# autonomousvision/unimatch

Hardware: AMD Instinct MI355X
Metric: image_pairs_per_sec (higher is better)
Workload: dtype f16x2

## Files before the change

### unimatch_amd/build.py

```python
import os
import re
import shutil
import subprocess
import sys

HERE = os.path.dirname(os.path.abspath(__file__))
CSRC = os.path.join(HERE, 'csrc')
LIB = os.path.join(HERE, 'libunimatch_hip.so')
SOURCES = ['capi.hip', 'global_match.hip', 'window_attn.hip', 'local_ops.hip', 'linear.hip', 'ffn.hip', 'conv.hip', 'nhwc_ops.hip', 'norm_ops.hip', 'upsample.hip',
           'rccl_gather.hip', 'local_corr_mfma.hip', 'aliases.hip', 'probe.hip', 'video.hip', 'metrics.hip', 'prepost.hip', 'visualize.hip']
DIAG_SOURCES = ['microbench.hip']
HEADERS = ['common.h', 'planes.h', 'timing.h', os.path.join('..', '..', 'include', 'unimatch_hip.h')]
EXTRA_FLAGS = {'ffn.hip': ['-fno-slp-vectorize'], 'global_match.hip': ['-fno-slp-vectorize', '-mllvm', '-amdgpu-mfma-vgpr-form', '-Wno-inline-asm'], 'window_attn.hip': ['-fno-slp-vectorize'],
               'linear.hip': ['-fno-slp-vectorize'],
               'video.hip': ['-ffp-contract=off'],
               'metrics.hip': ['-ffp-contract=off', '-fhip-fp32-correctly-rounded-divide-sqrt'],
               'prepost.hip': ['-ffp-contract=off', '-fhip-fp32-correctly-rounded-divide-sqrt'],
               'visualize.hip': ['-ffp-contract=off', '-fhip-fp32-correctly-rounded-divide-sqrt']}
RESOURCE_GUARDS = {'conv.hip': {'conv_entry_kernel': 2}}
FLAGS = ['--offload-arch=gfx950', '-O3', '-std=c++17', '-fPIC', '-fno-gpu-rdc', '-Wno-unused-result']


def find_hipcc():
    for cand in (os.environ.get('HIPCC'), shutil.which('hipcc'), '/opt/rocm/bin/hipcc'):
        if cand and os.path.exists(cand):
            return cand
    raise RuntimeError('hipcc not found: the HIP extension cannot be built')


def parse_resource_report(text):
    out, cur = {}, None
    for line in text.splitlines():
        m = re.search(r'remark: .*?Function Name: (\S+)', line)
        if m:
            cur = out.setdefault(m.group(1), {})
            continue
        m = re.search(r'remark: .*?\s{2,}([A-Za-z ]+?)(?: \[[^\]]*\])?: (\d+)', line)
        if m and cur is not None:
            cur[m.group(1).strip()] = int(m.group(2))
    return out


def check_resources(src, report):
    for key, min_occ in RESOURCE_GUARDS.get(src, {}).items():
        hits = {k: v for k, v in report.items() if key in k}
        if not hits:
            raise RuntimeError(f'{src}: no resource report for {key}: the guard of unimatch_amd/build.py has nothing to check')
        for name, r in hits.items():
            if r.get('ScratchSize', -1) != 0 or r.get('Occupancy', 0) < min_occ:
                raise RuntimeError(f'{src}: {name} needs scratch {r.get("ScratchSize")} B/lane at occupancy {r.get("Occupancy")} '
                                   f'({r.get("VGPRs")} VGPRs): it was written for no scratch at {min_occ} waves per SIMD')


def _stale(target, deps):
    if not os.path.exists(target):
        return True
    t = os.path.getmtime(target)
    return any(os.path.getmtime(d) > t for d in deps)


def build(force=False, verbose=False):
    hipcc = find_hipcc()
    objdir = os.path.join(HERE, '_obj')
    os.makedirs(objdir, exist_ok=True)
    hdrs = [os.path.normpath(os.path.join(CSRC, h)) for h in HEADERS] + [os.path.abspath(__file__)]
    objs = []
    for src in SOURCES:
        s = os.path.join(CSRC, src)
        o = os.path.join(objdir, src.replace('.hip', '.o'))
        if force or _stale(o, [s] + hdrs) or (src in RESOURCE_GUARDS and not os.path.exists(o[:-2] + '.resources.txt')):
            cmd = [hipcc] + FLAGS + EXTRA_FLAGS.get(src, []) + ['-c', s, '-o', o]
            if verbose:
                print(' '.join(cmd))
            if src in RESOURCE_GUARDS:
                done = subprocess.run(cmd + ['-Rpass-analysis=kernel-resource-usage', '-fno-caret-diagnostics'], cwd=CSRC, stderr=subprocess.PIPE, text=True)
                remarks = [ln for ln in done.stderr.splitlines() if 'kernel-resource-usage' in ln]
                sys.stderr.write('\n'.join(ln for ln in done.stderr.splitlines() if 'kernel-resource-usage' not in ln))
                if done.returncode != 0:
                    raise subprocess.CalledProcessError(done.returncode, cmd)
                try:
                    check_resources(src, parse_resource_report('\n'.join(remarks)))
                except RuntimeError:
                    os.remove(o)
                    raise
                with open(o[:-2] + '.resources.txt', 'w') as f:
                    f.write('\n'.join(remarks) + '\n')
            else:
                subprocess.run(cmd, check=True, cwd=CSRC)
        objs.append(o)
    if force or _stale(LIB, objs):
        cmd = [hipcc, '--offload-arch=gfx950', '-shared', '-fPIC', '-o', LIB] + objs + ['-ldl']
        if verbose:
            print(' '.join(cmd))
        subprocess.run(cmd, check=True)
    return LIB


def build_variant(name, defines, verbose=False, only=None):
    hipcc = find_hipcc()
    objdir = os.path.join(HERE, '_variants', '_obj_' + name)
    os.makedirs(objdir, exist_ok=True)
    objs = []
    defines = list(defines) + ['-DUM_DIAGNOSTIC_BUILD']
    if only:
        build(verbose=verbose)
    for src in SOURCES + DIAG_SOURCES:
        if only and src not in only and src not in DIAG_SOURCES:
            objs.append(os.path.join(HERE, '_obj', src.replace('.hip', '.o')))
            continue
        o = os.path.join(objdir, src.replace('.hip', '.o'))
        cmd = [hipcc] + FLAGS + EXTRA_FLAGS.get(src, []) + list(defines) + ['-c', os.path.join(CSRC, src), '-o', o]
        if verbose:
            print(' '.join(cmd))
        subprocess.run(cmd, check=True, cwd=CSRC)
        objs.append(o)
    lib = os.path.join(HERE, '_variants', f'lib{name}.so')
    subprocess.run([hipcc, '--offload-arch=gfx950', '-shared', '-fPIC', '-o', lib] + objs + ['-ldl'], check=True)
    shutil.rmtree(objdir, ignore_errors=True)
    return lib


if __name__ == '__main__':
    if '--variant' in sys.argv:
        i = sys.argv.index('--variant')
        only = sys.argv[sys.argv.index('--only') + 1].split(',') if '--only' in sys.argv else None
        print(build_variant(sys.argv[i + 1], [a for a in sys.argv[i + 2:] if a.startswith('-D')], verbose=True, only=only))
    else:
        print(build(force='--force' in sys.argv, verbose=True))
```

### unimatch_amd/csrc/conv.hip

```cpp
#include <cstdlib>
#include <cstring>
#ifndef UM_CONV_2P
#define UM_CONV_2P 0
#endif
#include "common.h"
#include "planes.h"

struct ConvArgs {
    const unsigned short* ap;
    long a_plane_stride;
    unsigned row_stride;
    unsigned zero_row;
    const unsigned short* wp;
    long w_plane_stride;
    const float* bias;
    float* out;
    unsigned short* outp;
    long outp_plane_stride;
    int out_ld, out_coff, outp_ld, outp_coff;
    int act;
    int gate, gate_c, gate_zld;
    float* gate_h;
    const float* gate_z;
    float* gate_hout;
// ... 447 lines not shown
    __syncthreads();

    int ptap = 0, pcc = 0;
    for (int s = 0; s < nstage; ++s) {
        unsigned char* cur = lds + (s & 1) * STAGE;
        unsigned char* nxt = lds + ((s & 1) ^ 1) * STAGE;
        const bool centre = ENTRY && ptap == 4;
        if constexpr (ENTRY) {
            if (centre) proj_load(pcc, 0);
        }
        if (s + 1 < nstage) {
            stage_async(cc * 32, (s + 1) * 32, nxt);
            if constexpr (ENTRY) entry_load(cc * 32);
            advance();
        }
        const unsigned char* at = cur + 32 * wave * 64;
        const unsigned char* wt = cur + NS * TILE;
        __builtin_amdgcn_s_setprio(1);
#pragma unroll
        for (int ks = 0; ks < 2; ++ks) {
            const i16x8 bh = *reinterpret_cast<const i16x8*>(at + foff[ks]);
            i16x8 bl;
            if (NS == 2) bl = *reinterpret_cast<const i16x8*>(at + TILE + foff[ks]);
#pragma unroll
            for (int nt = 0; nt < NT; ++nt) {
                const i16x8 wh = *reinterpret_cast<const i16x8*>(wt + nt * 32 * 64 + foff[ks]);
                if (NS == 2) {
                    const i16x8 wl = *reinterpret_cast<const i16x8*>(wt + WTILE + nt * 32 * 64 + foff[ks]);
                    if (UM_CONV_2P != 1) acc[nt] = T::mfma(wl, bh, acc[nt]);
                    if (UM_CONV_2P != 2) acc[nt] = T::mfma(wh, bl, acc[nt]);
                }
                acc[nt] = T::mfma(wh, bh, acc[nt]);
            }
            if constexpr (ENTRY) {
                if (centre) {
#pragma unroll
                    for (int nt = 0; nt < NT; ++nt) {
                        if (NS == 2) {
                            if (UM_CONV_2P != 1) acc2[nt] = T::mfma(pwl[nt], bh, acc2[nt]);
                            if (UM_CONV_2P != 2) acc2[nt] = T::mfma(pwh[nt], bl, acc2[nt]);
                        }
                        acc2[nt] = T::mfma(pwh[nt], bh, acc2[nt]);
                    }
                    if (ks == 0) proj_load(pcc, 1);
                }
            }
        }
        __builtin_amdgcn_s_setprio(0);
        if constexpr (ENTRY) {
            if (s + 1 < nstage) entry_store(nxt);
            if (++pcc == cpt) {
                pcc = 0;
                ++ptap;
            }
        }
        asm volatile("s_waitcnt vmcnt(0)" ::: "memory");
        __syncthreads();
    }

    {
        const int rloc0 = pl0 + 32 * wave;
        conv_epilogue<T, NS, NT, NT, !ENTRY>(a, acc, lds, lds + RING, bt, rloc0, min(32, max(0, P - rloc0)), bt * ((P + 127) / 128) + pl0 / 128, false,
                                 n0, tid, wave, lane, half);
        if constexpr (ENTRY) {
            ConvArgs a2 = a;
            a2.bias = e.bias2;
            a2.out = e.out2;
            a2.stats = e.stats2;
            __syncthreads();
            conv_epilogue<T, NS, NT, NT, false>(a2, acc2, lds, lds + RING, bt, rloc0, min(32, max(0, P - rloc0)), bt * ((P + 127) / 128) + pl0 / 128,
                                     false, n0, tid, wave, lane, half);
        }
    }
}

template <typename T, int NS, int NT>
__global__ __launch_bounds__(256, 2) void conv_kernel(ConvArgs a) {
    __shared__ __attribute__((aligned(16))) unsigned char lds[ConvLds<NS, NT>::TOTAL];
    conv_body<T, NS, NT, false>(a, ConvEntryArgs{}, lds);
}

template <typename T, int NS, int NT>
__global__ __launch_bounds__(256, 2) void conv_entry_kernel(ConvArgs a, ConvEntryArgs e) {
    __shared__ __attribute__((aligned(16))) unsigned char lds[ConvLds<NS, NT>::ENTRY_TOTAL];
    conv_body<T, NS, NT, true>(a, e, lds);
}

template <int NS, int NT, int KW, int NSLOT>
struct ConvRowsLds {
    static constexpr int NTE = NT < 2 ? NT : 2;
    static constexpr int ATILE = 288 * 32;
    static constexpr int WTILE = 32 * NT * 32;
    static constexpr int STAGE = NS * (ATILE + KW * WTILE);
    static constexpr int EPI = 8 * 32 * (32 * NTE * 4);
    static constexpr int RING = (NSLOT * STAGE > EPI) ? NSLOT * STAGE : EPI;
    static constexpr int TOTAL = RING + 8 * 2 * 32 * NT * 4 + 64;
};

__device__ __forceinline__ void conv_wait_vm(int n) {
    switch (n) {
        case 0: asm volatile("s_waitcnt vmcnt(0)" ::: "memory"); break;
        case 1: asm volatile("s_waitcnt vmcnt(1)" ::: "memory"); break;
        case 2: asm volatile("s_waitcnt vmcnt(2)" ::: "memory"); break;
        case 3: asm volatile("s_waitcnt vmcnt(3)" ::: "memory"); break;
        case 4: asm volatile("s_waitcnt vmcnt(4)" ::: "memory"); break;
        case 6: asm volatile("s_waitcnt vmcnt(6)" ::: "memory"); break;
        case 8: asm volatile("s_waitcnt vmcnt(8)" ::: "memory"); break;
        case 9: asm volatile("s_waitcnt vmcnt(9)" ::: "memory"); break;
        case 12: asm volatile("s_waitcnt vmcnt(12)" ::: "memory"); break;
        case 16: asm volatile("s_waitcnt vmcnt(16)" ::: "memory"); break;
        case 18: asm volatile("s_waitcnt vmcnt(18)" ::: "memory"); break;
        case 24: asm volatile("s_waitcnt vmcnt(24)" ::: "memory"); break;
        default: asm volatile("s_waitcnt vmcnt(0)" ::: "memory"); break;
    }
}

template <typename T, int NS, int NT, int KW, int NSLOT>
__global__ __launch_bounds__(512, (NSLOT == 2 && NT < 4 ? 2 : 1)) void conv_rows_kernel(ConvArgs a) {
    using L = ConvRowsLds<NS, NT, KW, NSLOT>;
    constexpr int ATILE = L::ATILE, WTILE = L::WTILE, STAGE = L::STAGE, RING = L::RING;
    extern __shared__ __attribute__((aligned(16))) unsigned char lds[];

    const int tid = threadIdx.x, lane = tid & 63;
    const int wave = __builtin_amdgcn_readfirstlane(tid >> 6);
    const int half = lane >> 5, fr = lane & 31;
    const int P = a.Ho * a.Wo, tpi = (P + 255) / 256;
    const int ny = (a.Cout + 32 * NT - 1) / (32 * NT);
    const int wg = a.xcd ? xcd_remap(blockIdx.x, gridDim.x) : blockIdx.x;
    const int tile = wg / ny;
    const int bt = tile / tpi, pl0 = (tile - bt * tpi) * 256;
    const int n0 = (wg - tile * ny) * (32 * NT);
    const int cpt = a.Cin >> 4;
    const int nstage = a.KH * cpt;
    const int ktot = a.KH * KW * a.Cin;

    const int dcp = lane & 1;
    int wy[2];
    long wflat[2];
    bool wok[2];
#pragma unroll
    for (int i = 0; i < 2; ++i) {
        const int jr = i == 0 ? wave : 8;
        const int j = 32 * jr + (lane >> 1);
        const int p = pl0 + j - a.pad_w;
        wok[i] = (i == 0 || wave == 7) && p >= 0 && p < P;
        const int rem = wok[i] ? p : 0;
        wy[i] = rem / a.Wo - a.pad_h;
        wflat[i] = (long)bt * P + rem - (long)a.pad_h * a.Wi;
    }
    unsigned rowoff[2];
    auto set_ky = [&](int ky) {
#pragma unroll
        for (int i = 0; i < 2; ++i) {
            const int iy = wy[i] + ky;
            const bool ok = wok[i] && (unsigned)iy < (unsigned)a.Hi;
            const unsigned row = ok ? (unsigned)(wflat[i] + (long)ky * a.Wi) : a.zero_row;
            rowoff[i] = row * a.row_stride;
        }
    };
    constexpr int NPIECE = 2 + (KW * NT + 7) / 8;
    auto stage_piece = [&](int k, int ky, int cc, unsigned char* buf) {
        if (k < 2) {
            const int jr = k == 0 ? wave : 8;
            if (k == 0 || wave == 7) {
                const int r = 32 * jr + (lane >> 1);
                const int sc = dcp ^ ((r >> 3) & 1);
                const unsigned off = rowoff[k] + (unsigned)((cc * 16 + 8 * sc) * 2);
#pragma unroll
                for (int pl = 0; pl < NS; ++pl) conv_dma16(a.ap + pl * a.a_plane_stride, off, buf + pl * ATILE + (32 * jr) * 32);
            }
        } else {
            const int q = wave + 8 * (k - 2);
            if (q < KW * NT) {
                const int kx = q / NT, jb = q - kx * NT;
                const int r = 32 * jb + (lane >> 1);
                const int sc = dcp ^ ((r >> 3) & 1);
                const int n = min(n0 + r, a.Cout - 1);
                const unsigned off = (unsigned)(((long)n * ktot + (ky * KW + kx) * a.Cin + cc * 16 + 8 * sc) * 2);
#pragma unroll
                for (int pl = 0; pl < NS; ++pl)
                    conv_dma16(a.wp + pl * a.w_plane_stride, off, buf + NS * ATILE + (kx * NS + pl) * WTILE + (32 * jb) * 32);
            }
        }
    };

    bool tap_ok[KW];
    bool any_masked = false;
    {
        const int p = pl0 + 32 * wave + fr;
        const bool pok = p < P;
        const int x = (pok ? p : 0) % a.Wo;
#pragma unroll
        for (int kx = 0; kx < KW; ++kx) {
            tap_ok[kx] = pok && (unsigned)(x + kx - a.pad_w) < (unsigned)a.Wi;
            any_masked |= !tap_ok[kx];
        }
    }
    const bool wave_masked = __any(any_masked);

    f32x16 acc[NT];
#pragma unroll
    for (int nt = 0; nt < NT; ++nt)
#pragma unroll
        for (int r = 0; r < 16; ++r) acc[nt][r] = 0.f;

    const int foffw = fr * 32 + ((half ^ ((fr >> 3) & 1)) << 4);
    int foffa[KW];
#pragma unroll
    for (int kx = 0; kx < KW; ++kx) {
        const int r = 32 * wave + fr + kx;
        foffa[kx] = r * 32 + ((half ^ ((r >> 3) & 1)) << 4);
    }

    int cnt = NS * (1 + (wave == 7 ? 1 : 0));
#pragma unroll
    for (int k = 2; k < NPIECE; ++k) cnt += (wave + 8 * (k - 2) < KW * NT) ? NS : 0;
    constexpr int D = NSLOT - 1;

    int ky = 0, cc = 0;
    set_ky(0);
    auto advance = [&]() {
        if (++cc == cpt) {
            cc = 0;
            ++ky;
            set_ky(ky);
        }
    };
#pragma unroll
    for (int d = 0; d < D; ++d)
        if (d < nstage) {
#pragma unroll
            for (int k = 0; k < NPIECE; ++k) stage_piece(k, ky, cc, lds + d * STAGE);
            advance();
        }
    conv_wait_vm(nstage >= D ? cnt * (D - 1) : 0);
    __syncthreads();

    int cur_off = 0, nxt_off = D * STAGE;
    for (int s = 0; s < nstage; ++s) {
        unsigned char* cur = lds + cur_off;
        unsigned char* nxt = lds + nxt_off;
        const bool more = s + D < nstage;
        __builtin_amdgcn_s_setprio(1);
#pragma unroll
        for (int kx = 0; kx < KW; ++kx) {
            const unsigned char* wt = cur + NS * ATILE + kx * NS * WTILE;
            if (more) {
                constexpr int GROUPS = KW - 1;
#pragma unroll
                for (int k = 0; k < NPIECE; ++k)
                    if (k % GROUPS == kx && kx < GROUPS) stage_piece(k, ky, cc, nxt);
            }
            i16x8 bh = *reinterpret_cast<const i16x8*>(cur + foffa[kx]);
            i16x8 bl;
            if (NS == 2) bl = *reinterpret_cast<const i16x8*>(cur + ATILE + foffa[kx]);
            if (wave_masked && !tap_ok[kx]) {
                const i16x8 z = {0, 0, 0, 0, 0, 0, 0, 0};
                bh = z;
                bl = z;
            }
#pragma unroll
            for (int nt = 0; nt < NT; ++nt) {
                const i16x8 wh = *reinterpret_cast<const i16x8*>(wt + nt * 32 * 32 + foffw);
                if (NS == 2) {
                    const i16x8 wl = *reinterpret_cast<const i16x8*>(wt + WTILE + nt * 32 * 32 + foffw);
                    if (UM_CONV_2P != 1) acc[nt] = T::mfma(wl, bh, acc[nt]);
                    if (UM_CONV_2P != 2) acc[nt] = T::mfma(wh, bl, acc[nt]);
                }
                acc[nt] = T::mfma(wh, bh, acc[nt]);
            }
        }
        __builtin_amdgcn_s_setprio(0);
        if (more) advance();
        conv_wait_vm(more ? cnt * (D - 1) : 0);
        __syncthreads();
        cur_off = cur_off + STAGE == NSLOT * STAGE ? 0 : cur_off + STAGE;
        nxt_off = nxt_off + STAGE == NSLOT * STAGE ? 0 : nxt_off + STAGE;
    }
    {
        const int rloc0 = pl0 + 32 * wave;
        conv_epilogue<T, NS, NT, L::NTE>(a, acc, lds, lds + RING, bt, rloc0, min(32, max(0, P - rloc0)), bt * ((P + 127) / 128) + pl0 / 128,
                                         false, n0, tid, wave, lane, half);
    }
}


template <int NS, int NT>
struct ConvPatchLds {
    static constexpr int NTE = NT < 2 ? NT : 2;
    static constexpr int PW = 34, PPIX = 10 * PW;
    static constexpr int PROWS = 352;
    static constexpr int ATILE = PROWS * 32;
    static constexpr int WTILE = 32 * NT * 32;
    static constexpr int ASLOT = NS * ATILE, WSLOT = NS * 3 * WTILE;
    static constexpr int WBASE = 2 * ASLOT;
    static constexpr int STAGES = 2 * ASLOT + 2 * WSLOT;
    static constexpr int EPI = 8 * 32 * (32 * NTE * 4);
    static constexpr int SCRATCH = 8 * 2 * 32 * NT * 4 + 64;
    static constexpr int TOTAL = (STAGES > EPI + SCRATCH) ? STAGES : EPI + SCRATCH;
};

typedef const __attribute__((address_space(4))) float* um_const_f32p;

template <typename T, int NS, int NT, bool NORM>
__device__ __forceinline__ void conv_patch_body(const ConvArgs& a, unsigned char* lds) {
    using L = ConvPatchLds<NS, NT>;
    constexpr int ATILE = L::ATILE, WTILE = L::WTILE, ASLOT = L::ASLOT, WSLOT = L::WSLOT, WBASE = L::WBASE;
    constexpr int PW = L::PW;

    const int tid = threadIdx.x, lane = tid & 63;
    const int wave = __builtin_amdgcn_readfirstlane(tid >> 6);
    const int half = lane >> 5, fr = lane & 31;
    const int twn = (a.Wo + 31) >> 5, tpi = twn * ((a.Ho + 7) >> 3);
    const int ny = (a.Cout + 32 * NT - 1) / (32 * NT);
    const int wg = a.xcd ? xcd_remap(blockIdx.x, gridDim.x) : blockIdx.x;
    const int tile = wg / ny;
    const int bt = tile / tpi, tt = tile - bt * tpi;
    const int ty = tt / twn, tx = tt - ty * twn;
    const int y0 = ty * 8, x0 = tx * 32;
    const int n0 = (wg - tile * ny) * (32 * NT);
    const int cpt = a.Cin >> 4;
    const int ktot = 9 * a.Cin;

    const int dcp = lane & 1;
    unsigned rowoff[2];
#pragma unroll
    for (int i = 0; i < 2; ++i) {
        const int j = 32 * (wave + 8 * i) + (lane >> 1);
        const int py = j / PW, px = j - py * PW;
        const int iy = y0 - 1 + py, ix = x0 - 1 + px;
        const bool ok = j < L::PPIX && (unsigned)iy < (unsigned)a.Hi && (unsigned)ix < (unsigned)a.Wi;
        if constexpr (NORM) {
            rowoff[i] = ok ? (unsigned)((bt * a.Hi + iy) * a.Wi + ix) * (unsigned)(a.Cin * 4) : ~0u;
        } else {
            const unsigned row = ok ? (unsigned)((bt * a.Hi + iy) * a.Wi + ix) : a.zero_row;
            rowoff[i] = row * a.row_stride;
        }
    }
    auto stage_patch = [&](int cc, unsigned char* buf) {
#pragma unroll
        for (int i = 0; i < 2; ++i)
            if (i == 0 || wave < 3) {
                const int blk = wave + 8 * i;
                const int r = 32 * blk + (lane >> 1);
                const int sc = dcp ^ ((r >> 3) & 1);
                const unsigned off = rowoff[i] + (unsigned)((cc * 16 + 8 * sc) * 2);
#pragma unroll
                for (int pl = 0; pl < NS; ++pl) conv_dma16(a.ap + pl * a.a_plane_stride, off, buf + pl * ATILE + (32 * blk) * 32);
            }
    };
    const int nsc = dcp ^ ((lane >> 4) & 1);
    f32x4 nx0, nx1;
    auto norm_load = [&](int cc, int i) {
        const unsigned off = (rowoff[i] == ~0u ? 0u : rowoff[i]) + (unsigned)((cc * 16 + 8 * nsc) * 4);
        const unsigned char* p = reinterpret_cast<const unsigned char*>(a.xf) + off;
        nx0 = *reinterpret_cast<const f32x4*>(p);
        nx1 = *reinterpret_cast<const f32x4*>(p + 16);
    };
    auto norm_store = [&](int cc, int i, unsigned char* buf) {
        const um_const_f32p mu = (um_const_f32p)(unsigned long)(a.nstats + ((long)bt * 2) * a.Cin + cc * 16);
        const um_const_f32p rs = mu + a.Cin;
        float v[8];
#pragma unroll
        for (int k = 0; k < 8; ++k) {
            const float m = nsc ? mu[8 + k] : mu[k], r = nsc ? rs[8 + k] : rs[k];
            v[k] = ((k < 4 ? nx0[k & 3] : nx1[k & 3]) - m) * r;
        }
        if (a.norm_relu) {
#pragma unroll
            for (int k = 0; k < 8; ++k) v[k] = fmaxf(v[k], 0.f);
        }
        const bool ok = rowoff[i] != ~0u;
        u32x4 h = {T::pack2(v[0], v[1]), T::pack2(v[2], v[3]), T::pack2(v[4], v[5]), T::pack2(v[6], v[7])};
        unsigned char* dst = buf + (32 * (wave + 8 * i)) * 32 + lane * 16;
        if (NS == 2) {
            u32x4 l;
#pragma unroll
            for (int k = 0; k < 4; ++k) {
                const f32x2 u = T::unpack2(h[k]);
                l[k] = ok ? T::pack2(v[2 * k] - u[0], v[2 * k + 1] - u[1]) : 0u;
            }
            *reinterpret_cast<u32x4*>(dst + ATILE) = l;
        }
#pragma unroll
        for (int k = 0; k < 4; ++k) h[k] = ok ? h[k] : 0u;
        *reinterpret_cast<u32x4*>(dst) = h;
    };
    auto stage_w = [&](int cc, int ky, unsigned char* buf) {
#pragma unroll
        for (int k = 0; k < (3 * NT + 7) / 8; ++k) {
            const int q = wave + 8 * k;
            if (q < 3 * NT) {
                const int kx = q / NT, jb = q - kx * NT;
                const int r = 32 * jb + (lane >> 1);
                const int sc = dcp ^ ((r >> 3) & 1);
                const int n = min(n0 + r, a.Cout - 1);
                const unsigned off = (unsigned)(((long)n * ktot + (ky * 3 + kx) * a.Cin + cc * 16 + 8 * sc) * 2);
#pragma unroll
                for (int pl = 0; pl < NS; ++pl)
                    conv_dma16(a.wp + pl * a.w_plane_stride, off, buf + (kx * NS + pl) * WTILE + (32 * jb) * 32);
            }
        }
    };

    f32x16 acc[NT];
#pragma unroll
    for (int nt = 0; nt < NT; ++nt)
#pragma unroll
        for (int r = 0; r < 16; ++r) acc[nt][r] = 0.f;

    const int foffw = fr * 32 + ((half ^ ((fr >> 3) & 1)) << 4);
    int foffa[3][3];
#pragma unroll
    for (int ky = 0; ky < 3; ++ky)
#pragma unroll
        for (int kx = 0; kx < 3; ++kx) {
            const int r = (wave + ky) * PW + kx + fr;
            foffa[ky][kx] = r * 32 + ((half ^ ((r >> 3) & 1)) << 4);
        }

    if constexpr (NORM) {
        stage_w(0, 0, lds + WBASE);
        norm_load(0, 0);
        norm_store(0, 0, lds);
        if (wave < 3) {
            norm_load(0, 1);
            norm_store(0, 1, lds);
        }
    } else {
        stage_patch(0, lds);
        stage_w(0, 0, lds + WBASE);
    }
    asm volatile("s_waitcnt vmcnt(0)" ::: "memory");
    __syncthreads();

    for (int cc = 0; cc < cpt; ++cc) {
        const int a_cur = (cc & 1) * ASLOT, a_nxt = ASLOT - a_cur;
#pragma unroll
        for (int ky = 0; ky < 3; ++ky) {
            const int w_par = (cc + ky) & 1;
            const int w_cur = WBASE + w_par * WSLOT, w_nxt = WBASE + (w_par ^ 1) * WSLOT;
            const bool last = ky == 2 && cc + 1 == cpt;
            __builtin_amdgcn_s_setprio(1);
#pragma unroll
            for (int kx = 0; kx < 3; ++kx) {
                if (kx == 0 && !last) stage_w(ky == 2 ? cc + 1 : cc, ky == 2 ? 0 : ky + 1, lds + w_nxt);
                if constexpr (NORM) {
                    if (kx == 1 && cc + 1 < cpt) {
                        if (ky == 0) norm_load(cc + 1, 0);
                        if (ky == 1) {
                            norm_store(cc + 1, 0, lds + a_nxt);
                            if (wave < 3) norm_load(cc + 1, 1);
                        }
                        if (ky == 2 && wave < 3) norm_store(cc + 1, 1, lds + a_nxt);
                    }
                } else {
                    if (kx == 1 && ky == 0 && cc + 1 < cpt) stage_patch(cc + 1, lds + a_nxt);
                }
                const i16x8 bh = *reinterpret_cast<const i16x8*>(lds + a_cur + foffa[ky][kx]);
                i16x8 bl;
                if (NS == 2) bl = *reinterpret_cast<const i16x8*>(lds + a_cur + ATILE + foffa[ky][kx]);
                const unsigned char* wt = lds + w_cur + kx * NS * WTILE;
#pragma unroll
                for (int nt = 0; nt < NT; ++nt) {
                    const i16x8 wh = *reinterpret_cast<const i16x8*>(wt + nt * 32 * 32 + foffw);
                    if (NS == 2) {
                        const i16x8 wl = *reinterpret_cast<const i16x8*>(wt + WTILE + nt * 32 * 32 + foffw);
                        if (UM_CONV_2P != 1) acc[nt] = T::mfma(wl, bh, acc[nt]);
                        if (UM_CONV_2P != 2) acc[nt] = T::mfma(wh, bl, acc[nt]);
                    }
                    acc[nt] = T::mfma(wh, bh, acc[nt]);
                }
            }
            __builtin_amdgcn_s_setprio(0);
            asm volatile("s_waitcnt vmcnt(0)" ::: "memory");
            __syncthreads();
        }
    }
    const int nvalid = y0 + wave < a.Ho ? min(32, a.Wo - x0) : 0;
    conv_epilogue<T, NS, NT, L::NTE>(a, acc, lds, lds + L::EPI, bt, (y0 + wave) * a.Wo + x0, nvalid, (bt * tpi + tt) * 2, true, n0, tid,
                                     wave, lane, half);
}

template <typename T, int NS, int NT>
__global__ __launch_bounds__(512, (NT < 4 ? 2 : 1)) void conv_patch_kernel(ConvArgs a) {
    extern __shared__ __attribute__((aligned(16))) unsigned char lds[];
    conv_patch_body<T, NS, NT, false>(a, lds);
}

template <typename T, int NS, int NT>
__global__ __launch_bounds__(512, (NT < 4 ? 2 : 1)) void conv_patch_norm_kernel(ConvArgs a) {
    extern __shared__ __attribute__((aligned(16))) unsigned char lds[];
    conv_patch_body<T, NS, NT, true>(a, lds);
}

extern void um_set_error(const char* fmt, ...);

static int conv_xcd_enabled() {
    static const int on = um_debug_env("UM_CONV_NO_XCD") == nullptr;
    return on;
}

template <int NT>
static hipError_t launch_conv(const ConvArgs& a, int mode, hipStream_t stream) {
    dim3 grid(a.B * ((a.Ho * a.Wo + 127) / 128) * ((a.Cout + 32 * NT - 1) / (32 * NT))), block(256);
    ScopedKernelTimer timer(UM_K_CONV, stream);
    um_census_hit(UM_V_CONV_GENERIC);
    if (mode == 0)
        hipLaunchKernelGGL((conv_kernel<Fp16, 2, NT>), grid, block, 0, stream, a);
    else
        hipLaunchKernelGGL((conv_kernel<Bf16, 1, NT>), grid, block, 0, stream, a);
    return hipGetLastError();
}

template <int NT>
static hipError_t launch_conv_entry(const ConvArgs& a, const ConvEntryArgs& e, int mode, hipStream_t stream) {
    dim3 grid(a.B * ((a.Ho * a.Wo + 127) / 128) * ((a.Cout + 32 * NT - 1) / (32 * NT))), block(256);
    ScopedKernelTimer timer(UM_K_CONV, stream);
    um_census_hit(UM_V_CONV_GENERIC);
    if (mode == 0)
        hipLaunchKernelGGL((conv_entry_kernel<Fp16, 2, NT>), grid, block, 0, stream, a, e);
    else
        hipLaunchKernelGGL((conv_entry_kernel<Bf16, 1, NT>), grid, block, 0, stream, a, e);
    return hipGetLastError();
}

template <int NT, int KW, int NSLOT>
static hipError_t launch_conv_rows(const ConvArgs& a, int mode, hipStream_t stream) {
    static bool configured[2] = {false, false};
    dim3 grid(a.B * ((a.Ho * a.Wo + 255) / 256) * ((a.Cout + 32 * NT - 1) / (32 * NT))), block(512);
    constexpr int LDS2 = ConvRowsLds<2, NT, KW, NSLOT>::TOTAL, LDS1 = ConvRowsLds<1, NT, KW, NSLOT>::TOTAL;
    static_assert(LDS2 <= 160 * 1024 && LDS1 <= 160 * 1024, "ring beyond the CU's LDS");
    ScopedKernelTimer timer(UM_K_CONV, stream);
    um_census_hit(UM_V_CONV_ROWS);
    if (mode == 0) {
        if (!configured[0]) {
            hipError_t e = hipFuncSetAttribute(reinterpret_cast<const void*>(&conv_rows_kernel<Fp16, 2, NT, KW, NSLOT>),
                                               hipFuncAttributeMaxDynamicSharedMemorySize, LDS2);
            if (e != hipSuccess) return e;
            configured[0] = true;
        }
        hipLaunchKernelGGL((conv_rows_kernel<Fp16, 2, NT, KW, NSLOT>), grid, block, LDS2, stream, a);
    } else {
        if (!configured[1]) {
            hipError_t e = hipFuncSetAttribute(reinterpret_cast<const void*>(&conv_rows_kernel<Bf16, 1, NT, KW, NSLOT>),
                                               hipFuncAttributeMaxDynamicSharedMemorySize, LDS1);
            if (e != hipSuccess) return e;
            configured[1] = true;
        }
        hipLaunchKernelGGL((conv_rows_kernel<Bf16, 1, NT, KW, NSLOT>), grid, block, LDS1, stream, a);
    }
    return hipGetLastError();
}

template <int NT, bool NORM = false>
static hipError_t launch_conv_patch(const ConvArgs& a, int mode, hipStream_t stream) {
    static bool configured[2] = {false, false};
    dim3 grid(a.B * ((a.Ho + 7) / 8) * ((a.Wo + 31) / 32) * ((a.Cout + 32 * NT - 1) / (32 * NT))), block(512);
    constexpr int LDS2 = ConvPatchLds<2, NT>::TOTAL, LDS1 = ConvPatchLds<1, NT>::TOTAL;
    static_assert(LDS2 <= 160 * 1024 && LDS1 <= 160 * 1024, "ring beyond the CU's LDS");
    ScopedKernelTimer timer(UM_K_CONV, stream);
    um_census_hit(UM_V_CONV_PATCH);
    if (NORM) um_census_hit(UM_V_CONV_PATCH_NORM);
    void (*k2)(ConvArgs), (*k1)(ConvArgs);
    if constexpr (NORM) {
        k2 = conv_patch_norm_kernel<Fp16, 2, NT>;
        k1 = conv_patch_norm_kernel<Bf16, 1, NT>;
    } else {
        k2 = conv_patch_kernel<Fp16, 2, NT>;
        k1 = conv_patch_kernel<Bf16, 1, NT>;
    }
    if (mode == 0) {
        if (!configured[0]) {
            hipError_t e = hipFuncSetAttribute(reinterpret_cast<const void*>(k2), hipFuncAttributeMaxDynamicSharedMemorySize, LDS2);
            if (e != hipSuccess) return e;
            configured[0] = true;
        }
        hipLaunchKernelGGL(k2, grid, block, LDS2, stream, a);
    } else {
        if (!configured[1]) {
            hipError_t e = hipFuncSetAttribute(reinterpret_cast<const void*>(k1), hipFuncAttributeMaxDynamicSharedMemorySize, LDS1);
            if (e != hipSuccess) return e;
            configured[1] = true;
        }
        hipLaunchKernelGGL(k1, grid, block, LDS1, stream, a);
    }
    return hipGetLastError();
}

enum ConvKind { CONV_GENERIC = 0, CONV_ROWS = 1, CONV_PATCH = 2 };

static ConvKind conv_pick(int hi, int wi, int ho, int wo, int cout, int kh, int kw, int stride, int pad_h, int pad_w, int* nt_out) {
    const int nt = (cout % 128 == 0 || cout > 192) ? 4 : (cout % 96 == 0) ? 3 : (cout <= 64 || cout % 64 == 0) ? 2 : 4;
    *nt_out = nt;
    static const bool rows_enabled = um_debug_env("UM_CONV_NO_ROWS") == nullptr;
    static const char* patch_env = um_debug_env("UM_CONV_PATCH");
    static const char* patch_nts = patch_env ? patch_env : "234";
    const bool same = stride == 1 && ho == hi && wo == wi && (long)ho * wo >= 256 && rows_enabled;
    const bool rows3 = same && kw == 3 && pad_w == 1, rows5 = same && kw == 5 && pad_w == 2 && nt == 4;
    const long tiled = (long)((ho + 7) / 8 * 8) * ((wo + 31) / 32 * 32);
    if (rows3 && kh == 3 && pad_h == 1 && 4L * ho * wo >= 3 * tiled && strchr(patch_nts, '0' + nt) != nullptr) {
        if (cout <= 32) *nt_out = 1;
        return CONV_PATCH;
    }
    return rows3 || rows5 ? CONV_ROWS : CONV_GENERIC;
}

static constexpr bool kNormOnLoad[5] = {false, false, true, true, true};

extern "C" int um_conv2d_norm_supported(int hi, int wi, int cin, int cout, int kh, int kw, int stride, int pad_h, int pad_w, int mode) {
    if (hi <= 0 || wi <= 0 || cin <= 0 || cin % 32 != 0 || cout <= 0 || cout % 4 != 0 || kh <= 0 || kw <= 0 || stride <= 0 || pad_h < 0 ||
        pad_w < 0 || (mode != 0 && mode != 1))
        return 0;
    const int ho = (hi + 2 * pad_h - kh) / stride + 1, wo = (wi + 2 * pad_w - kw) / stride + 1;
    if (ho <= 0 || wo <= 0) return 0;
    int nt;
    if (conv_pick(hi, wi, ho, wo, cout, kh, kw, stride, pad_h, pad_w, &nt) != CONV_PATCH) return 0;
    return nt >= 2 && nt <= 4 && kNormOnLoad[nt] ? 1 : 0;
}

static constexpr bool kEntryConv[5] = {false, false, false, true, true};

extern "C" int um_conv2d_entry_supported(int hi, int wi, int cin, int cout, int kh, int kw, int stride, int pad_h, int pad_w, int mode) {
    if (hi <= 0 || wi <= 0 || cin <= 0 || cin % 32 != 0 || cin > ConvLds<2, 4>::ENTRY_CIN || cout <= 0 || cout % 4 != 0 ||
        (mode != 0 && mode != 1))
        return 0;
    if (kh != 3 || kw != 3 || stride != 2 || pad_h != 1 || pad_w != 1) return 0;
    const int ho = (hi - 1) / 2 + 1, wo = (wi - 1) / 2 + 1;
    int nt;
    if (conv_pick(hi, wi, ho, wo, cout, 3, 3, 2, 1, 1, &nt) != CONV_GENERIC) return 0;
    return nt >= 3 && nt <= 4 && kEntryConv[nt] ? 1 : 0;
}

extern "C" int um_conv_stats_parts(int hi, int wi, int cout, int kh, int kw, int stride, int pad_h, int pad_w) {
    if (hi <= 0 || wi <= 0 || cout <= 0 || kh <= 0 || kw <= 0 || stride <= 0 || pad_h < 0 || pad_w < 0) return -1;
    const int ho = (hi + 2 * pad_h - kh) / stride + 1, wo = (wi + 2 * pad_w - kw) / stride + 1;
    if (ho <= 0 || wo <= 0) return -1;
    int nt;
    if (conv_pick(hi, wi, ho, wo, cout, kh, kw, stride, pad_h, pad_w, &nt) == CONV_PATCH) return 2 * ((ho + 7) / 8) * ((wo + 31) / 32);
    return (int)(((long)ho * wo + 127) / 128);
}

static int conv2d_impl(const void* a_planes, int a_ld, int a_coff, long a_rows, const void* w_planes, const float* bias,
                       float* out, int out_ld, int out_coff, void* out_planes, int outp_ld, int outp_coff, long outp_rows,
                       float* stats_out, int batch, int hi, int wi, int cin, int cout, int kh, int kw, int stride,
                       int pad_h, int pad_w, int act, int wshift, int mode, void* stream_, int gate, float* gate_h,
                       const float* gate_z, int gate_zld, const float* addend = nullptr, int addend_ld = 0, float* gate_hout = nullptr,
                       int gate_hout_ld = 0, const float* norm_x = nullptr, const float* norm_stats = nullptr, int norm_relu = 0,
                       int addend_period = 0) {
    const bool norm = norm_x != nullptr;
    if (gate_hout && (gate != 2 || gate_hout_ld < cout || gate_hout_ld % 4 != 0 || ((unsigned long)gate_hout & 15) != 0)) {
        um_set_error("um_conv2d: a separate new-state tensor goes with gate 2 only: 16-byte aligned fp32 [M][ld >= channels, ld %% 4 == 0]");
        return -1;
    }
    if (addend && (addend_ld < cout || addend_ld % 4 != 0 || ((unsigned long)addend & 15) != 0 || stats_out)) {
        um_set_error("um_conv2d: the addend must be 16-byte aligned fp32 [M][ld >= cout, ld %% 4 == 0] (and excludes fused statistics)");
        return -1;
    }
    if ((!a_planes && !norm) || !w_planes || (!out && !out_planes) || batch <= 0 || hi <= 0 || wi <= 0 || cin <= 0 || cin % 32 != 0 ||
        cout <= 0 || cout % 4 != 0 || kh <= 0 || kw <= 0 || stride <= 0 || pad_h < 0 || pad_w < 0 || (mode != 0 && mode != 1) ||
        wshift < 0 || wshift > 14 || act < 0 || act > 3) {
        um_set_error("um_conv2d: bad argument (batch=%d hi=%d wi=%d cin=%d cout=%d k=%dx%d stride=%d pad=%d,%d act=%d; cin must "
                     "be a multiple of 32, cout of 4)", batch, hi, wi, cin, cout, kh, kw, stride, pad_h, pad_w, act);
        return -1;
    }
    const int ho = (hi + 2 * pad_h - kh) / stride + 1, wo = (wi + 2 * pad_w - kw) / stride + 1;
    if (ho <= 0 || wo <= 0) {
        um_set_error("um_conv2d: empty output (%d x %d)", ho, wo);
        return -1;
    }
    const long rows_in = (long)batch * hi * wi, m = (long)batch * ho * wo;
    if (a_ld < a_coff + cin || a_ld % 8 != 0 || a_coff % 8 != 0 || a_rows < rows_in + 1 ||
        (out && (out_ld < out_coff + cout || out_ld % 4 != 0 || out_coff % 4 != 0)) ||
        (out_planes && (outp_ld < outp_coff + (gate == 1 ? cout / 2 : cout) || outp_ld % 4 != 0 || outp_coff % 4 != 0 ||
                        outp_rows < m))) {
        um_set_error("um_conv2d: inconsistent leading dimensions / offsets / row counts");
        return -1;
    }
    if (stats_out && !out) {
        um_set_error("um_conv2d: fused statistics need the fp32 output");
        return -1;
    }
    if (bias && ((unsigned long)bias & 15) != 0) {
        um_set_error("um_conv2d: bias must be 16-byte aligned");
        return -1;
    }
    if (a_rows * a_ld * 2 >= (1L << 32) || (long)cout * kh * kw * cin * 2 >= (1L << 32) || m >= (1L << 31)) {
        um_set_error("um_conv2d: operand planes beyond 4 GiB are not addressable by this kernel");
        return -4;
    }
    if (norm) {
        if (!norm_stats || ((unsigned long)norm_x & 15) != 0 || ((unsigned long)norm_stats & 3) != 0) {
            um_set_error("um_conv2d_norm_fwd: the fp32 input must be 16-byte aligned and comes with its statistics [batch][2][cin]");
            return -1;
        }
        if (!um_conv2d_norm_supported(hi, wi, cin, cout, kh, kw, stride, pad_h, pad_w, mode)) {
            um_set_error("um_conv2d_norm_fwd: no on-load kernel for this geometry (hi=%d wi=%d cin=%d cout=%d k=%dx%d stride=%d pad=%d,%d): "
                         "ask um_conv2d_norm_supported() first", hi, wi, cin, cout, kh, kw, stride, pad_h, pad_w);
            return -2;
        }
        if (rows_in * cin * 4 >= (1L << 32) - 1) {
            um_set_error("um_conv2d_norm_fwd: an fp32 input beyond 4 GiB is not addressable by this kernel");
            return -4;
        }
    }
    ConvArgs a;
    a.xf = norm_x;
    a.nstats = norm_stats;
    a.norm_relu = norm_relu;
    a.ap = (const unsigned short*)a_planes + a_coff;
    a.a_plane_stride = a_rows * a_ld;
    a.row_stride = (unsigned)a_ld * 2;
    a.zero_row = (unsigned)(a_rows - 1);
    a.wp = (const unsigned short*)w_planes;
    a.w_plane_stride = (long)cout * kh * kw * cin;
    a.bias = bias;
    a.out = out;
    a.out_ld = out_ld;
    a.out_coff = out_coff;
    a.outp = (unsigned short*)out_planes;
    a.outp_ld = outp_ld;
    a.outp_coff = outp_coff;
    a.outp_plane_stride = outp_rows * outp_ld;
    a.stats = stats_out;
    a.addend = addend;
    a.addend_ld = addend_ld;
    a.addend_period = addend_period;
    a.B = batch;
    a.Hi = hi;
    a.Wi = wi;
    a.Cin = cin;
    a.Ho = ho;
    a.Wo = wo;
    a.Cout = cout;
    a.KH = kh;
    a.KW = kw;
    a.stride = stride;
    a.pad_h = pad_h;
    a.pad_w = pad_w;
    a.M = (int)m;
    a.act = act;
    a.gate = gate;
    a.gate_c = gate == 1 ? cout / 2 : cout;
    a.gate_h = gate_h;
    a.gate_z = gate_z;
    a.gate_zld = gate_zld;
    a.gate_hout = gate_hout ? gate_hout : gate_h;
    a.gate_hout_ld = gate_hout ? gate_hout_ld : a.gate_c;
    a.out_scale = ldexpf(1.f, -wshift);
    a.xcd = conv_xcd_enabled();
    hipError_t e;
    int nt;
    const ConvKind kind = conv_pick(hi, wi, ho, wo, cout, kh, kw, stride, pad_h, pad_w, &nt);
    hipStream_t st = (hipStream_t)stream_;
    if (norm)
        e = nt == 2 ? launch_conv_patch<2, true>(a, mode, st) : nt == 3 ? launch_conv_patch<3, true>(a, mode, st) : launch_conv_patch<4, true>(a, mode, st);
    else if (kind == CONV_PATCH)
        e = nt == 1 ? launch_conv_patch<1>(a, mode, st) : nt == 2 ? launch_conv_patch<2>(a, mode, st) : nt == 3 ? launch_conv_patch<3>(a, mode, st)
                                                                                                          : launch_conv_patch<4>(a, mode, st);
    else if (kind == CONV_ROWS && kw == 5) e = launch_conv_rows<4, 5, 2>(a, mode, st);
    else if (kind == CONV_ROWS) e = nt == 2 ? launch_conv_rows<2, 3, 2>(a, mode, st) : nt == 3 ? launch_conv_rows<3, 3, 2>(a, mode, st) : launch_conv_rows<4, 3, 2>(a, mode, st);
    else e = nt == 2 ? launch_conv<2>(a, mode, st) : nt == 3 ? launch_conv<3>(a, mode, st) : launch_conv<4>(a, mode, st);
    if (e != hipSuccess) {
        um_set_error("um_conv2d: launch failed: %s", hipGetErrorString(e));
        return (int)e;
    }
    return 0;
}

extern "C" int um_conv2d_ex(const void* a_planes, int a_ld, int a_coff, long a_rows, const void* w_planes, const float* bias,
                            float* out, int out_ld, int out_coff, void* out_planes, int outp_ld, int outp_coff, long outp_rows,
                            float* stats_out, int batch, int hi, int wi, int cin, int cout, int kh, int kw, int stride,
                            int pad_h, int pad_w, int act, int wshift, int mode, void* stream_) {
    return conv2d_impl(a_planes, a_ld, a_coff, a_rows, w_planes, bias, out, out_ld, out_coff, out_planes, outp_ld, outp_coff,
                       outp_rows, stats_out, batch, hi, wi, cin, cout, kh, kw, stride, pad_h, pad_w, act, wshift, mode, stream_, 0,
                       nullptr, nullptr, 0);
}

extern "C" int um_conv2d_gru_fwd(int gate, const void* a_planes, int a_ld, int a_coff, long a_rows, const void* w_planes,
                                 const float* bias, float* hidden, const float* z, int z_ld, float* z_out, int z_out_ld,
// ... 303 lines not shown
```

Before: 966.2.

## Software-pipeline LDS fragment loads and DMA staging in wide-N conv patch kernel

Adds a pipelined main loop for the 3x3 patch convolution kernels with NT of 3 or 4. It double-buffers operand fragments in registers, prefetching the next weight and patch fragments while MFMAs run, and uses sched_group_barrier to interleave LDS reads with MFMA. It also replaces full vmcnt(0) waits plus syncthreads with partial waits and a raw s_barrier, and issues paired two-plane DMA with precomputed scalar LDS addresses. The extra fragment registers put occupancy at risk, so the build guard now checks occupancy and scratch for several instantiations.

New measurement: 972.6 (median of 6 runs). No clear change (+0.7%).

```diff
diff --git a/unimatch_amd/build.py b/unimatch_amd/build.py
--- a/unimatch_amd/build.py
+++ b/unimatch_amd/build.py
@@ -17,7 +17,10 @@
                'metrics.hip': ['-ffp-contract=off', '-fhip-fp32-correctly-rounded-divide-sqrt'],
                'prepost.hip': ['-ffp-contract=off', '-fhip-fp32-correctly-rounded-divide-sqrt'],
                'visualize.hip': ['-ffp-contract=off', '-fhip-fp32-correctly-rounded-divide-sqrt']}
-RESOURCE_GUARDS = {'conv.hip': {'conv_entry_kernel': 2}}
+RESOURCE_GUARDS = {'conv.hip': {'conv_entry_kernel': 2,
+                                **{f'{kernel}I4{arith}ELi{nt}EE': 4
+                                   for kernel in ('conv_patch_kernel', 'conv_patch_norm_kernel')
+                                   for arith in ('Fp16Li2', 'Bf16Li1') for nt in (2, 3)}}}
 FLAGS = ['--offload-arch=gfx950', '-O3', '-std=c++17', '-fPIC', '-fno-gpu-rdc', '-Wno-unused-result']
 
 
@@ -41,15 +44,21 @@
     return out
 
 
-def check_resources(src, report):
+def check_resources(src, report, require_all=False):
+    checked = False
     for key, min_occ in RESOURCE_GUARDS.get(src, {}).items():
         hits = {k: v for k, v in report.items() if key in k}
         if not hits:
-            raise RuntimeError(f'{src}: no resource report for {key}: the guard of unimatch_amd/build.py has nothing to check')
+            if require_all:
+                raise RuntimeError(f'{src}: no resource report for {key}: the guard of unimatch_amd/build.py has nothing to check')
+            continue
+        checked = True
         for name, r in hits.items():
             if r.get('ScratchSize', -1) != 0 or r.get('Occupancy', 0) < min_occ:
                 raise RuntimeError(f'{src}: {name} needs scratch {r.get("ScratchSize")} B/lane at occupancy {r.get("Occupancy")} '
                                    f'({r.get("VGPRs")} VGPRs): it was written for no scratch at {min_occ} waves per SIMD')
+    if RESOURCE_GUARDS.get(src) and not checked:
+        raise RuntimeError(f'{src}: no resource report for any guarded kernel: the guard of unimatch_amd/build.py has nothing to check')
 
 
 def _stale(target, deps):
@@ -79,7 +88,7 @@
                 if done.returncode != 0:
                     raise subprocess.CalledProcessError(done.returncode, cmd)
                 try:
-                    check_resources(src, parse_resource_report('\n'.join(remarks)))
+                    check_resources(src, parse_resource_report('\n'.join(remarks)), require_all=True)
                 except RuntimeError:
                     os.remove(o)
                     raise
diff --git a/unimatch_amd/csrc/conv.hip b/unimatch_amd/csrc/conv.hip
--- a/unimatch_amd/csrc/conv.hip
+++ b/unimatch_amd/csrc/conv.hip
@@ -773,15 +773,56 @@
 
 typedef const __attribute__((address_space(4))) float* um_const_f32p;
 
+#if defined(UM_CONV_PATCH_PIPE_OFF)
+static constexpr bool kPatchPipe[5] = {false, false, false, false, false};
+#elif defined(UM_CONV_PATCH_PIPE_ALL)
+static constexpr bool kPatchPipe[5] = {false, true, true, true, true};
+#else
+static constexpr bool kPatchPipe[5] = {false, false, false, true, true};
+#endif
+
+__device__ __forceinline__ void conv_dma16(const void* base, unsigned byte_off, unsigned lds_addr) {
+    lds_addr = __builtin_amdgcn_readfirstlane(lds_addr);
+    unsigned keep;
+    asm volatile("s_mov_b32 %0, m0\n\ts_mov_b32 m0, %3\n\ts_nop 0\n\tglobal_load_lds_dwordx4 %1, %2\n\ts_mov_b32 m0, %0"
+                 : "=&s"(keep)
+                 : "v"(byte_off), "s"(base), "s"(lds_addr)
+                 : "memory");
+}
+__device__ __forceinline__ void conv_dma16x2(const void* base0, const void* base1, unsigned byte_off, unsigned lds_addr0, unsigned lds_addr1) {
+    lds_addr0 = __builtin_amdgcn_readfirstlane(lds_addr0);
+    lds_addr1 = __builtin_amdgcn_readfirstlane(lds_addr1);
+    unsigned keep;
+    asm volatile("s_mov_b32 %0, m0\n\ts_mov_b32 m0, %4\n\ts_nop 0\n\tglobal_load_lds_dwordx4 %1, %2\n\t"
+                 "s_mov_b32 m0, %5\n\ts_nop 0\n\tglobal_load_lds_dwordx4 %1, %3\n\ts_mov_b32 m0, %0"
+                 : "=&s"(keep)
+                 : "v"(byte_off), "s"(base0), "s"(base1), "s"(lds_addr0), "s"(lds_addr1)
+                 : "memory");
+}
+
 template <typename T, int NS, int NT, bool NORM>
 __device__ __forceinline__ void conv_patch_body(const ConvArgs& a, unsigned char* lds) {
     using L = ConvPatchLds<NS, NT>;
     constexpr int ATILE = L::ATILE, WTILE = L::WTILE, ASLOT = L::ASLOT, WSLOT = L::WSLOT, WBASE = L::WBASE;
     constexpr int PW = L::PW;
+    constexpr bool PIPE = kPatchPipe[NT];
 
     const int tid = threadIdx.x, lane = tid & 63;
     const int wave = __builtin_amdgcn_readfirstlane(tid >> 6);
     const int half = lane >> 5, fr = lane & 31;
+    const unsigned ldsb = __builtin_amdgcn_readfirstlane((unsigned)(unsigned long)(const __attribute__((address_space(3))) unsigned char*)lds);
+    auto ring = [&](int off) {
+        if constexpr (PIPE) return ldsb + (unsigned)off;
+        else return lds + off;
+    };
+    auto dma_planes = [&](const unsigned short* base, long plane_stride, unsigned off, auto dst, int dst_plane) {
+        if constexpr (PIPE && NS == 2) {
+            conv_dma16x2(base, base + plane_stride, off, dst, dst + dst_plane);
+        } else {
+#pragma unroll
+            for (int pl = 0; pl < NS; ++pl) conv_dma16(base + pl * plane_stride, off, dst + pl * dst_plane);
+        }
+    };
     const int twn = (a.Wo + 31) >> 5, tpi = twn * ((a.Ho + 7) >> 3);
     const int ny = (a.Cout + 32 * NT - 1) / (32 * NT);
     const int wg = a.xcd ? xcd_remap(blockIdx.x, gridDim.x) : blockIdx.x;
@@ -808,7 +849,7 @@
             rowoff[i] = row * a.row_stride;
         }
     }
-    auto stage_patch = [&](int cc, unsigned char* buf) {
+    auto stage_patch = [&](int cc, auto buf) {
 #pragma unroll
         for (int i = 0; i < 2; ++i)
             if (i == 0 || wave < 3) {
@@ -816,8 +857,7 @@
                 const int r = 32 * blk + (lane >> 1);
                 const int sc = dcp ^ ((r >> 3) & 1);
                 const unsigned off = rowoff[i] + (unsigned)((cc * 16 + 8 * sc) * 2);
-#pragma unroll
-                for (int pl = 0; pl < NS; ++pl) conv_dma16(a.ap + pl * a.a_plane_stride, off, buf + pl * ATILE + (32 * blk) * 32);
+                dma_planes(a.ap, a.a_plane_stride, off, buf + (32 * blk) * 32, ATILE);
             }
     };
     const int nsc = dcp ^ ((lane >> 4) & 1);
@@ -857,7 +897,7 @@
         for (int k = 0; k < 4; ++k) h[k] = ok ? h[k] : 0u;
         *reinterpret_cast<u32x4*>(dst) = h;
     };
-    auto stage_w = [&](int cc, int ky, unsigned char* buf) {
+    auto stage_w = [&](int cc, int ky, auto buf) {
 #pragma unroll
         for (int k = 0; k < (3 * NT + 7) / 8; ++k) {
             const int q = wave + 8 * k;
@@ -867,9 +907,7 @@
                 const int sc = dcp ^ ((r >> 3) & 1);
                 const int n = min(n0 + r, a.Cout - 1);
                 const unsigned off = (unsigned)(((long)n * ktot + (ky * 3 + kx) * a.Cin + cc * 16 + 8 * sc) * 2);
-#pragma unroll
-                for (int pl = 0; pl < NS; ++pl)
-                    conv_dma16(a.wp + pl * a.w_plane_stride, off, buf + (kx * NS + pl) * WTILE + (32 * jb) * 32);
+                dma_planes(a.wp, a.w_plane_stride, off, buf + kx * NS * WTILE + (32 * jb) * 32, WTILE);
             }
         }
     };
@@ -891,7 +929,7 @@
         }
 
     if constexpr (NORM) {
-        stage_w(0, 0, lds + WBASE);
+        stage_w(0, 0, ring(WBASE));
         norm_load(0, 0);
         norm_store(0, 0, lds);
         if (wave < 3) {
@@ -899,12 +937,82 @@
             norm_store(0, 1, lds);
         }
     } else {
-        stage_patch(0, lds);
-        stage_w(0, 0, lds + WBASE);
+        stage_patch(0, ring(0));
+        stage_w(0, 0, ring(WBASE));
     }
     asm volatile("s_waitcnt vmcnt(0)" ::: "memory");
     __syncthreads();
 
+    if constexpr (PIPE) {
+    i16x8 fb[3][NS], fw[2][NS];
+    auto ld_b = [&](int slot, int a_off, int ky, int kx) {
+#pragma unroll
+        for (int pl = 0; pl < NS; ++pl) fb[slot][pl] = *reinterpret_cast<const i16x8*>(lds + a_off + pl * ATILE + foffa[ky][kx]);
+    };
+    auto ld_w = [&](int slot, int w_off, int u) {
+        const int kx = u / NT, nt = u - kx * NT;
+#pragma unroll
+        for (int pl = 0; pl < NS; ++pl)
+            fw[slot][pl] = *reinterpret_cast<const i16x8*>(lds + w_off + (kx * NS + pl) * WTILE + nt * 32 * 32 + foffw);
+    };
+    const int n_patch = NORM ? 2 : NS * (wave < 3 ? 2 : 1);
+    if constexpr (!NORM) ld_b(0, 0, 0, 0);
+    for (int cc = 0; cc < cpt; ++cc) {
+        const int a_cur = (cc & 1) * ASLOT, a_nxt = ASLOT - a_cur;
+        const bool more = cc + 1 < cpt;
+#pragma unroll
+        for (int ky = 0; ky < 3; ++ky) {
+            const int w_par = (cc + ky) & 1;
+            const int w_cur = WBASE + w_par * WSLOT, w_nxt = WBASE + (w_par ^ 1) * WSLOT;
+            const bool last = ky == 2 && !more;
+            __builtin_amdgcn_s_setprio(1);
+            if (NORM && ky == 0) ld_b(0, a_cur, 0, 0);
+            ld_w(0, w_cur, 0);
+            __builtin_amdgcn_sched_barrier(0);
+#pragma unroll
+            for (int u = 0; u < 3 * NT; ++u) {
+                const int kx = u / NT, nt = u - kx * NT;
+                if constexpr (NORM) {
+                    if (nt == 0 && kx == 0 && ky == 0) stage_w(cc, 1, ring(w_nxt));
+                    if (nt == 0 && kx == 1) {
+                        if (more) {
+                            if (ky == 0) norm_load(cc + 1, 0);
+                            if (ky == 1) norm_store(cc + 1, 0, lds + a_nxt);
+                            if (ky == 2 && wave < 3) norm_store(cc + 1, 1, lds + a_nxt);
+                        }
+                        if (ky == 1) {
+                            stage_w(cc, 2, ring(w_nxt));
+                            if (more && wave < 3) norm_load(cc + 1, 1);
+                        }
+                        if (ky == 2 && !last) stage_w(cc + 1, 0, ring(w_nxt));
+                    }
+                } else {
+                    if (nt == 0 && kx == 0 && !last) stage_w(ky == 2 ? cc + 1 : cc, ky == 2 ? 0 : ky + 1, ring(w_nxt));
+                    if (nt == 0 && kx == 1 && ky == 0 && more) stage_patch(cc + 1, ring(a_nxt));
+                }
+                if (nt == 0 && kx < 2) ld_b(kx + 1, a_cur, ky, kx + 1);
+                if (u + 1 < 3 * NT) ld_w((u + 1) & 1, w_cur, u + 1);
+                else if (ky < 2) ld_b(0, a_cur, ky + 1, 0);
+                else if (!NORM) ld_b(0, a_nxt, 0, 0);
+                if (NS == 2) {
+                    if (UM_CONV_2P != 1) acc[nt] = T::mfma(fw[u & 1][NS - 1], fb[kx][0], acc[nt]);
+                    if (UM_CONV_2P != 2) acc[nt] = T::mfma(fw[u & 1][0], fb[kx][NS - 1], acc[nt]);
+                }
+                acc[nt] = T::mfma(fw[u & 1][0], fb[kx][0], acc[nt]);
+                __builtin_amdgcn_sched_group_barrier(0x100, 2 * NS, 0);
+                __builtin_amdgcn_sched_group_barrier(0x008, NS + 1, 0);
+                __builtin_amdgcn_sched_barrier(0);
+            }
+            __builtin_amdgcn_s_setprio(0);
+            int leave = 0;
+            if (more && ky == 0) leave = n_patch;
+            if (NORM && more && ky == 1) leave = wave < 3 ? 2 : 0;
+            conv_wait_vm(leave);
+            if constexpr (NORM) asm volatile("s_waitcnt lgkmcnt(0)\n\ts_barrier" ::: "memory");
+            else asm volatile("s_barrier" ::: "memory");
+        }
+    }
+    } else {
     for (int cc = 0; cc < cpt; ++cc) {
         const int a_cur = (cc & 1) * ASLOT, a_nxt = ASLOT - a_cur;
 #pragma unroll
@@ -947,6 +1055,7 @@
             asm volatile("s_waitcnt vmcnt(0)" ::: "memory");
             __syncthreads();
         }
+    }
     }
     const int nvalid = y0 + wave < a.Ho ? min(32, a.Wo - x0) : 0;
     conv_epilogue<T, NS, NT, L::NTE>(a, acc, lds, lds + L::EPI, bt, (y0 + wave) * a.Wo + x0, nvalid, (bt * tpi + tt) * 2, true, n0, tid,
```
